# zchuning/repo

Measured on AMD Instinct MI355X. Metric: world-model+imagine updates/sec (B=50,L=50,64x64x3), higher is better.
Workload: dtype f32

## Files before the change

### repo_amd/csrc/dconv.h

```cpp
#pragma once
#include "vgemm.h"

namespace repo {

template <int BM_, int BN_, int CK_, int WM_, int WN_, int LDWPAD_ = 2>
struct DTile {
  static constexpr int BM = BM_, BN = BN_, CK = CK_, WM = WM_, WN = WN_, LDWPAD = LDWPAD_;
  static constexpr int TM = BM / (32 * WM), TN = BN / (32 * WN);
  static constexpr int NT = WM * WN * 64;
  static_assert(TM >= 1 && TN >= 1 && BM % (32 * WM) == 0 && BN % (32 * WN) == 0, "tile / wave grid mismatch");
};

#ifdef REPO_IGEMM_STAMPS
#define REPO_STAMP_FLUSH(nslices)                                              \
  do {                                                                         \
    REPO_STAMP(4);                                                             \
    if ((threadIdx.x & 63) == 0 && blockIdx.x % 16 == 0) {                     \
      for (int i_ = 0; i_ < 6; ++i_) atomicAdd(&g_igemm_stamps[i_], st_[i_]);  \
      atomicAdd(&g_igemm_stamps[6], 1ull);                                     \
      atomicAdd(&g_igemm_stamps[7], (unsigned long long)(nslices));            \
    }                                                                          \
  } while (0)
#else
#define REPO_STAMP_FLUSH(nslices)
#endif

__device__ __forceinline__ int xcd_tile(int b, int n) {
  const int q = n >> 3, r = n & 7, x = b & 7, i = b >> 3;
  return x * q + min(x, r) + i;
}

constexpr int cmin(int a, int b) { return a < b ? a : b; }
constexpr int cmax(int a, int b) { return a > b ? a : b; }

template <class InT>
struct Patch4;
template <>
struct Patch4<float> {
  typedef f32x4 raw_t;
  static constexpr int BYTES = 4;
  static __device__ __forceinline__ raw_t load(__amdgpu_buffer_rsrc_t r, unsigned off) {
    return __builtin_bit_cast(f32x4, __builtin_amdgcn_raw_buffer_load_b128(r, off, 0, 0));
  }
  static __device__ __forceinline__ f32x4 cvt(raw_t v) { return v; }
};
template <>
struct Patch4<uint8_t> {
  typedef unsigned raw_t;
  static constexpr int BYTES = 1;
  static __device__ __forceinline__ raw_t load(__amdgpu_buffer_rsrc_t r, unsigned off) {
    return __builtin_amdgcn_raw_buffer_load_b32(r, off, 0, 0);
  }
  static __device__ __forceinline__ f32x4 cvt(raw_t v) {
    f32x4 o;
    o[0] = pix_norm((uint8_t)(v & 0xff));
    o[1] = pix_norm((uint8_t)((v >> 8) & 0xff));
    o[2] = pix_norm((uint8_t)((v >> 16) & 0xff));
    o[3] = pix_norm((uint8_t)(v >> 24));
    return o;
  }
};

typedef unsigned u32x4s __attribute__((ext_vector_type(4)));

struct DownArgs {
  const void* big;
  const float* w;
  const float* bias;
  const float* aux;
  float* out;
  int nimg, epi;
  unsigned big_bytes, w_bytes;
  float* chan_part;
  unsigned char* cmask;
};

template <class G, class T>
__device__ __forceinline__ void dconv_down_epilogue(const DownArgs& p, float* lds, f32x16 (&acc)[T::TM][T::TN], int n0,
                                                    int m0, int Ntot) {
  constexpr int BM = T::BM, NT = T::NT, TM = T::TM, TN = T::TN;
  constexpr int EP = 36;
  const int tid = threadIdx.x;
  const int lane = tid & 63;
  const int wid = __builtin_amdgcn_readfirstlane(tid >> 6);
  const int wm = wid / T::WN, wn = wid % T::WN;
  const int li = lane & 31, lh = lane >> 5;
  __syncthreads();
  float* strip = lds + wid * 32 * EP;
  const __amdgpu_buffer_rsrc_t rout = make_rsrc(p.out, 4u * (unsigned)Ntot * G::CS);
  float csum[TM][4];
#pragma unroll
  for (int i = 0; i < TM; ++i)
#pragma unroll
    for (int q4 = 0; q4 < 4; ++q4) csum[i][q4] = 0.f;
  const __amdgpu_buffer_rsrc_t raux =
      make_rsrc((p.aux && p.epi != REPO_EPI_FILM_RELU) ? p.aux : p.out, (p.epi == REPO_EPI_MUL_MASK4 ? 1u : 4u) * (unsigned)Ntot * G::CS);
#pragma unroll
  for (int i = 0; i < TM; ++i)
#pragma unroll
    for (int j = 0; j < TN; ++j) {
#pragma unroll
      for (int r = 0; r < 16; ++r) strip[((r & 3) + 8 * (r >> 2) + 4 * lh) * EP + li] = acc[i][j][r];
      __builtin_amdgcn_wave_barrier();
      const int nb = n0 + (wn * TN + j) * 32, mt = m0 + (wm * TM + i) * 32;
#pragma unroll
      for (int pass = 0; pass < 4; ++pass) {
        const int ml = pass * 8 + (lane >> 3), q = lane & 7;
        const int m = mt + ml, n = nb + 4 * q;
        f32x4 v = *reinterpret_cast<const f32x4*>(strip + ml * EP + 4 * q);
        float qs = 0.f;
        if (m < G::CS && n < Ntot) {
          const float bv = p.bias ? p.bias[m] : 0.f;
          const int img = n / G::PS, pix = n % G::PS;
          const unsigned o = (unsigned)((img * G::CS + m) * G::PS + pix);
          if (pix + 3 < G::PS && n + 3 < Ntot) {
            f32x4 a4 = {1.f, 1.f, 1.f, 1.f};
            if (p.epi == REPO_EPI_MUL_DRELU) {
              a4 = __builtin_bit_cast(f32x4, __builtin_amdgcn_raw_buffer_load_b128(raux, 4u * o, 0, 0));
            } else if (p.epi == REPO_EPI_MUL_MASK4) {
              unsigned bits = (unsigned)__builtin_amdgcn_raw_buffer_load_b8(raux, o >> 2, 0, 0) >> (o & 3);
              if (o & 3) bits |= (unsigned)__builtin_amdgcn_raw_buffer_load_b8(raux, (o >> 2) + 1, 0, 0) << (4 - (o & 3));
#pragma unroll
              for (int e = 0; e < 4; ++e) a4[e] = (bits >> e) & 1u ? 1.f : 0.f;
            }
            float fsc = 1.f, fsh = 0.f;
            if (p.epi == REPO_EPI_FILM_RELU) {
              fsc = p.aux[(size_t)(2 * img) * G::CS + m];
              fsh = p.aux[(size_t)(2 * img + 1) * G::CS + m];
            }
#pragma unroll
            for (int e = 0; e < 4; ++e) {
              float x = v[e] + bv;
              if (p.epi == REPO_EPI_RELU) x = fmaxf(x, 0.f);
              else if (p.epi == REPO_EPI_MUL_DRELU || p.epi == REPO_EPI_MUL_MASK4) x = a4[e] > 0.f ? x : 0.f;
              else if (p.epi == REPO_EPI_FILM_RELU) x = fmaxf(fmaf(fsc, x, fsh), 0.f);
              v[e] = x;
            }
            qs = (v[0] + v[1]) + (v[2] + v[3]);
            __builtin_amdgcn_raw_buffer_store_b128(__builtin_bit_cast(u32x4s, v), rout, 4u * o, 0, 0);
          } else {
#pragma unroll
            for (int e = 0; e < 4; ++e) {
              const int ne = n + e;
              if (ne < Ntot) {
                const int oe = ((ne / G::PS) * G::CS + m) * G::PS + ne % G::PS;
                float x = v[e] + bv;
                if (p.epi == REPO_EPI_RELU) x = fmaxf(x, 0.f);
                else if (p.epi == REPO_EPI_FILM_RELU)
                  x = fmaxf(fmaf(p.aux[(size_t)(2 * (ne / G::PS)) * G::CS + m], x, p.aux[(size_t)(2 * (ne / G::PS) + 1) * G::CS + m]), 0.f);
                else if (p.epi == REPO_EPI_MUL_DRELU) x = p.aux[oe] > 0.f ? x : 0.f;
                else if (p.epi == REPO_EPI_MUL_MASK4)
                  x = (reinterpret_cast<const unsigned char*>(p.aux)[oe >> 2] >> (oe & 3)) & 1 ? x : 0.f;
                p.out[oe] = x;
                qs += x;
              }
            }
          }
        }
        if (p.chan_part) {
          qs += __shfl_xor(qs, 1, 64);
          qs += __shfl_xor(qs, 2, 64);
          qs += __shfl_xor(qs, 4, 64);
          csum[i][pass] += qs;
        }
      }
      if (p.cmask) {
        const int cq = lane >> 3, q = lane & 7;
        const int m4 = mt + 4 * cq, n = nb + 4 * q;
        if (m4 < G::CS && n < Ntot) {
          f32x4 rws[4];
          float bq[4];
#pragma unroll
          for (int c = 0; c < 4; ++c) {
            rws[c] = *reinterpret_cast<const f32x4*>(strip + (4 * cq + c) * EP + 4 * q);
            bq[c] = p.bias ? p.bias[m4 + c] : 0.f;
          }
#pragma unroll
          for (int e = 0; e < 4; ++e) {
            const int ne = n + e;
            if (ne < Ntot) {
              unsigned bits = 0;
#pragma unroll
              for (int c = 0; c < 4; ++c) bits |= (rws[c][e] + bq[c] > 0.f ? 1u : 0u) << c;
              p.cmask[((size_t)(ne / G::PS) * (G::CS / 4) + (m4 >> 2)) * G::PS + ne % G::PS] = (unsigned char)bits;
            }
          }
        }
      }
      __builtin_amdgcn_wave_barrier();
    }
  if (p.chan_part) {
    float* red = lds + (NT / 64) * 32 * EP;
    if ((lane & 7) == 0) {
#pragma unroll
      for (int i = 0; i < TM; ++i)
#pragma unroll
        for (int pass = 0; pass < 4; ++pass) red[wid * (TM * 32) + i * 32 + pass * 8 + (lane >> 3)] = csum[i][pass];
    }
    __syncthreads();
    if (tid < BM && m0 + tid < G::CS) {
      const int wmc = tid / (TM * 32), c = tid % (TM * 32);
      float t = 0.f;
#pragma unroll
      for (int x = 0; x < T::WN; ++x) t += red[(wmc * T::WN + x) * (TM * 32) + c];
      p.chan_part[(size_t)blockIdx.x * G::CS + m0 + tid] = t;
    }
  }
}

template <class G, class BigT, class T>
__global__ __launch_bounds__(T::NT) void dconv_down_kernel(DownArgs p) {
  constexpr int BM = T::BM, BN = T::BN, CK = T::CK, NT = T::NT, TM = T::TM, TN = T::TN;
  constexpr int KSL = CK * G::KK;
  constexpr int NSL = G::CB / CK;
  static_assert(G::CB % CK == 0 && KSL % 4 == 0, "channel chunk must divide CB and give k % 4 == 0");
  constexpr int LDW = BM + T::LDWPAD;
  constexpr int ROWS_FULL = 2 * (G::HS - 1) + G::KS;
  constexpr int LENFULL = (ROWS_FULL * G::WB + 3) & ~3;
  constexpr int NIMG_MAX = (BN - 1) / G::PS + 2;
  constexpr int PLMAX = cmin(NIMG_MAX * LENFULL,
                             ((2 * (BN / G::WS + 2) + NIMG_MAX * (G::KS - 2)) * G::WB + 4 * NIMG_MAX + 3) & ~3);
  constexpr int PLV = PLMAX / 4;
  constexpr int W_NV = BM * KSL / 4, W_KV = KSL / 4;
  constexpr int W_PER = (W_NV + NT - 1) / NT, P_PER = (CK * PLV + NT - 1) / NT;
  constexpr int NBUF = NSL > 1 ? 2 : 1;
  constexpr int EP = 36;
  __shared__ __attribute__((aligned(16))) float lds[cmax(NBUF * KSL * LDW + NBUF * CK * PLMAX, (NT / 64) * 32 * EP + (NT / 64) * TM * 32)];
  float* Wl = lds;
  float* Pl = lds + NBUF * KSL * LDW;

  const int tid = threadIdx.x;
  const int lane = tid & 63;
  const int wid = __builtin_amdgcn_readfirstlane(tid >> 6);
  const int wm = wid / T::WN, wn = wid % T::WN;
  const int li = lane & 31, lh = lane >> 5;

  const int Ntot = p.nimg * G::PS;
  const int n0 = xcd_tile(blockIdx.x, gridDim.x) * BN, m0 = blockIdx.y * BM;
  const int nlast = min(n0 + BN, Ntot) - 1;
  const int ia = n0 / G::PS, ib = nlast / G::PS;
  const int fa = (n0 % G::PS) / G::WS, lb = (nlast % G::PS) / G::WS;
  const int la_ = (ia == ib) ? lb : G::HS - 1;
  const int lenA = ((2 * (la_ - fa) + G::KS) * G::WB + 3) & ~3;
  auto span_start = [&](int i) __attribute__((always_inline)) { return i == ia ? 0 : lenA + (i - ia - 1) * LENFULL; };
  const int PL = span_start(ib) + (ib == ia ? lenA : ((2 * lb + G::KS) * G::WB + 3) & ~3);

  const __amdgpu_buffer_rsrc_t rbig = make_rsrc(p.big, p.big_bytes), rw = make_rsrc(p.w, p.w_bytes);

  unsigned woff[W_PER];
  int wlds[W_PER];
#pragma unroll
  for (int j = 0; j < W_PER; ++j) {
    const int v = tid + j * NT, kv = v % W_KV, m = v / W_KV;
    const bool act = (W_NV % NT == 0) || v < W_NV;
    woff[j] = act ? 4u * (unsigned)(min(m0 + m, G::CS - 1) * (G::CB * G::KK) + kv * 4) : kOobOffset;
    wlds[j] = act ? (kv * 4) * LDW + m : -1;
  }
  unsigned poff[P_PER];
  int plds[P_PER];
#pragma unroll
  for (int j = 0; j < P_PER; ++j) {
    const int v = tid + j * NT, c = v / PLV, q = (v % PLV) * 4;
    const bool act = c < CK && q < PL;
    int i, rel;
    if (q < lenA) {
      i = ia;
      rel = q;
    } else {
      i = ia + 1 + (q - lenA) / LENFULL;
      rel = (q - lenA) % LENFULL;
    }
    const int f = (i == ia) ? fa : 0;
    poff[j] = act ? (unsigned)Patch4<BigT>::BYTES * (unsigned)((i * G::CB + c) * G::PB + 2 * f * G::WB + rel)
                  : kOobOffset;
    plds[j] = act ? c * PLMAX + q : -1;
  }
  constexpr unsigned W_STEP = 4u * KSL, P_STEP = (unsigned)Patch4<BigT>::BYTES * CK * G::PB;

  int bbase[TN];
#pragma unroll
  for (int j = 0; j < TN; ++j) {
    const int n = min(n0 + (wn * TN + j) * 32 + li, Ntot - 1);
    const int i = n / G::PS, pix = n % G::PS;
    const int f = (i == ia) ? fa : 0;
    bbase[j] = span_start(i) + 2 * (pix / G::WS - f) * G::WB + 2 * (pix % G::WS);
  }
  int bbase1[TN];
#pragma unroll
  for (int j = 0; j < TN; ++j) bbase1[j] = bbase[j] + lh;
  const int abase = lh * LDW + wm * (TM * 32) + li;

  f32x16 acc[TM][TN];
#pragma unroll
  for (int i = 0; i < TM; ++i)
#pragma unroll
    for (int j = 0; j < TN; ++j)
#pragma unroll
      for (int r = 0; r < 16; ++r) acc[i][j][r] = 0.f;

  f32x4 rwv[W_PER];
  typename Patch4<BigT>::raw_t rpv[P_PER];
  auto gload = [&](int t) __attribute__((always_inline)) {
#pragma unroll
    for (int j = 0; j < W_PER; ++j)
      rwv[j] = VecLoad<4>::load(rw, woff[j] == kOobOffset ? kOobOffset : woff[j] + (unsigned)t * W_STEP);
#pragma unroll
    for (int j = 0; j < P_PER; ++j)
      rpv[j] = Patch4<BigT>::load(rbig, poff[j] == kOobOffset ? kOobOffset : poff[j] + (unsigned)t * P_STEP);
  };
  auto lstore = [&](int buf) __attribute__((always_inline)) {
    float* wl = Wl + buf * KSL * LDW;
    float* pl = Pl + buf * CK * PLMAX;
#pragma unroll
    for (int j = 0; j < W_PER; ++j)
      if ((W_NV % NT == 0) || wlds[j] >= 0) {
#pragma unroll
        for (int e = 0; e < 4; ++e) wl[wlds[j] + e * LDW] = rwv[j][e];
      }
#pragma unroll
    for (int j = 0; j < P_PER; ++j)
      if (plds[j] >= 0) *reinterpret_cast<f32x4*>(pl + plds[j]) = Patch4<BigT>::cvt(rpv[j]);
  };
  auto koff = [](int k) constexpr { return (k / G::KK) * PLMAX + ((k % G::KK) / G::KS) * G::WB + (k % G::KK) % G::KS; };
  auto compute = [&](int buf) __attribute__((always_inline)) {
    const float* wl = Wl + buf * KSL * LDW + abase;
    const float* pl = Pl + buf * CK * PLMAX;
#pragma unroll
    for (int ks = 0; ks < KSL / 2; ++ks) {
      const int o0 = koff(2 * ks), o1 = koff(2 * ks + 1);
      float av[TM], bv[TN];
#pragma unroll
      for (int i = 0; i < TM; ++i) av[i] = wl[2 * ks * LDW + i * 32];
#pragma unroll
      for (int j = 0; j < TN; ++j) bv[j] = (o1 == o0 + 1) ? pl[bbase1[j] + o0] : pl[bbase[j] + (lh ? o1 : o0)];
#pragma unroll
      for (int i = 0; i < TM; ++i)
#pragma unroll
        for (int j = 0; j < TN; ++j)
          acc[i][j] = __builtin_amdgcn_mfma_f32_32x32x2f32(av[i], bv[j], acc[i][j], 0, 0, 0);
    }
  };

  REPO_STAMP_DECL
  gload(0);
  lstore(0);
  __syncthreads();
  REPO_STAMP(5);
  if (NSL == 1) {
    compute(0);
  } else {
    int buf = 0;
    for (int t = 0; t < NSL; ++t) {
      gload(min(t + 1, NSL - 1));
      __builtin_amdgcn_sched_barrier(0);
      REPO_STAMP(0);
      compute(buf);
      __builtin_amdgcn_sched_barrier(0);
      REPO_STAMP(1);
      lstore(buf ^ 1);
      REPO_STAMP(2);
      __syncthreads();
      REPO_STAMP(3);
      buf ^= 1;
    }
  }

  dconv_down_epilogue<G, T>(p, lds, acc, n0, m0, Ntot);
  REPO_STAMP_FLUSH(NSL);
}

template <class G, class BigT, class T>
inline int launch_dconv_down(const DownArgs& a, hipStream_t s) {
  const long gx = ((long)a.nimg * G::PS + T::BN - 1) / T::BN, gy = (G::CS + T::BM - 1) / T::BM;
  hipLaunchKernelGGL((dconv_down_kernel<G, BigT, T>), dim3((unsigned)gx, (unsigned)gy), dim3(T::NT), 0, s, a);
  hipError_t e = hipGetLastError();
  return e == hipSuccess ? REPO_OK : (int)e;
}

struct WgradArgs {
  const float* small;
  const void* big;
  float* slab;
  int nimg, imgs_per_split, want_db;
  unsigned small_bytes, big_bytes;
  int nsplits_tw = 0;
  int want_dbig = 0;
};

template <int BM_, int BN_, int WM_, int WN_, int GI_, int RB_, int SPREAD_ = 0>
struct WTile {
  static constexpr int BM = BM_, BN = BN_, WM = WM_, WN = WN_, GI = GI_, RB = RB_, SPREAD = SPREAD_;
  static constexpr int TM = BM / (32 * WM), TN = BN / (32 * WN), NT = WM * WN * 64;
  static_assert(TM >= 1 && TN >= 1 && BM % (32 * WM) == 0 && BN % (32 * WN) == 0, "tile / wave grid mismatch");
};

constexpr int pitch4(int len) {
  int p = (len + 3) & ~3;
  return (p / 4) % 2 ? p : p + 4;
}

template <class G, class BigT, class T>
__global__ __launch_bounds__(T::NT) void dconv_wgrad_kernel(WgradArgs p) {
  constexpr int BM = T::BM, BN = T::BN, TM = T::TM, TN = T::TN, NT = T::NT, GI = T::GI, RB = T::RB;
  constexpr int NW = G::CB * G::KK;
  constexpr int NB = (G::HS + RB - 1) / RB;
  constexpr int BR = 2 * RB + G::KS - 2;
  constexpr int BRP = (G::WB % 64 == 0) ? G::WB + 4 : G::WB;
  constexpr int ALEN = RB * G::WS, BLEN = BR * BRP;
  constexpr int AP = pitch4(ALEN), BP = pitch4(BLEN);
  constexpr int CBT = cmin(G::CB, (BN + G::KK - 2) / G::KK + 1);
  constexpr int A_VPC = (ALEN + 3) / 4, B_VPC = (BR * G::WB + 3) / 4;
  constexpr int A_NV = GI * BM * A_VPC, B_NV = GI * CBT * B_VPC;
  constexpr int A_PER = (A_NV + NT - 1) / NT, B_PER = (B_NV + NT - 1) / NT;
  constexpr int SXP = (G::WS + 1) / 2;
  __shared__ __attribute__((aligned(16))) float lds[GI * BM * AP + GI * CBT * BP + 64];
  float* Al = lds;
  float* Bl = lds + GI * BM * AP;

  const int tid = threadIdx.x;
  const int lane = tid & 63;
  const int wid = __builtin_amdgcn_readfirstlane(tid >> 6);
  const int wm = wid / T::WN, wn = wid % T::WN;
  const int li = lane & 31, lh = lane >> 5;

  int bx = blockIdx.x, by = blockIdx.y, z = blockIdx.z;
  {
    const int tpz = gridDim.x * gridDim.y, gz = gridDim.z;
    const int L = bx + gridDim.x * (by + gridDim.y * z);
    const int full = (gz / 8) * 8 * tpz;
    if (L < full) {
      const int grp = L / (8 * tpz), r = L % (8 * tpz);
      const int t = r / 8;
      z = grp * 8 + r % 8;
      bx = t % (int)gridDim.x;
      by = t / (int)gridDim.x;
    }
  }
  const int n0 = bx * BN, m0 = by * BM;
  const int img_beg = z * p.imgs_per_split, img_end = min(p.nimg, img_beg + p.imgs_per_split);
  const int cbf = n0 / G::KK;
  const int ngrp = (img_end - img_beg + GI - 1) / GI;
  const int nch = ngrp * NB;

  const __amdgpu_buffer_rsrc_t rsm = make_rsrc(p.small, p.small_bytes), rbg = make_rsrc(p.big, p.big_bytes);

  int aoff[A_PER], boff[B_PER], ag[A_PER], bg[B_PER];
  int alds[A_PER], blds[B_PER];
#pragma unroll
  for (int j = 0; j < A_PER; ++j) {
    const int v = tid + j * NT, e4 = v % A_VPC, rm = v / A_VPC;
    const int m = rm % BM, g = rm / BM;
    const bool act = g < GI && m0 + m < G::CS;
    ag[j] = act ? g : 1 << 20;
    aoff[j] = (g * G::CS + m0 + m) * G::PS + e4 * 4;
    alds[j] = (g * BM + m) * AP + e4 * 4;
  }
#pragma unroll
  for (int j = 0; j < B_PER; ++j) {
    const int v = tid + j * NT, e4 = v % B_VPC, rc = v / B_VPC;
    const int c = rc % CBT, g = rc / CBT;
    const bool act = g < GI && cbf + c < G::CB;
    bg[j] = act ? g : 1 << 20;
    boff[j] = (g * G::CB + cbf + c) * G::PB + e4 * 4;
    blds[j] = (g * CBT + c) * BP + (BRP == G::WB ? e4 * 4 : (e4 * 4 / G::WB) * BRP + e4 * 4 % G::WB);
  }

  int abase[TM], bbase[TN];
#pragma unroll
  for (int i = 0; i < TM; ++i) abase[i] = ((wm * TM + i) * 32 + li) * AP + lh;
#pragma unroll
  for (int j = 0; j < TN; ++j) {
    const int n = min(n0 + (wn * TN + j) * 32 + li, NW - 1);
    const int cb = n / G::KK, r = n % G::KK;
    bbase[j] = (cb - cbf) * BP + (r / G::KS) * BRP + r % G::KS + 2 * lh;
  }

  f32x16 acc[TM][TN];
#pragma unroll
  for (int i = 0; i < TM; ++i)
#pragma unroll
    for (int j = 0; j < TN; ++j)
#pragma unroll
      for (int r = 0; r < 16; ++r) acc[i][j][r] = 0.f;
  float dbsum = 0.f;

  f32x4 rav[A_PER];
  typename Patch4<BigT>::raw_t rbv[B_PER];
  constexpr int NLD = A_PER + B_PER;
  int ld_img0 = 0, ld_abias = 0, ld_bbias = 0;
  auto gload_begin = [&](int c) __attribute__((always_inline)) {
    const int grp = c / NB, band = c % NB;
    const int r0 = band * RB;
    ld_img0 = img_beg + grp * GI;
    ld_abias = ld_img0 * G::CS * G::PS + r0 * G::WS;
    ld_bbias = ld_img0 * G::CB * G::PB + 2 * r0 * G::WB;
  };
  auto gload_piece = [&](int q) __attribute__((always_inline)) {
#pragma unroll
    for (int j = 0; j < A_PER; ++j)
      if (j == q)
        rav[j] = VecLoad<4>::load(rsm, ld_img0 + ag[j] < img_end ? 4u * (unsigned)(aoff[j] + ld_abias) : kOobOffset);
#pragma unroll
    for (int j = 0; j < B_PER; ++j)
      if (j + A_PER == q)
        rbv[j] = Patch4<BigT>::load(
            rbg, ld_img0 + bg[j] < img_end ? (unsigned)Patch4<BigT>::BYTES * (unsigned)(boff[j] + ld_bbias) : kOobOffset);
  };
  auto gload = [&](int c) __attribute__((always_inline)) {
    gload_begin(c);
#pragma unroll
    for (int q = 0; q < NLD; ++q) gload_piece(q);
  };
  auto lstore = [&]() __attribute__((always_inline)) {
#pragma unroll
    for (int j = 0; j < A_PER; ++j)
      if ((A_NV % NT == 0) || tid + j * NT < A_NV) *reinterpret_cast<f32x4*>(Al + alds[j]) = rav[j];
#pragma unroll
    for (int j = 0; j < B_PER; ++j)
      if ((B_NV % NT == 0) || tid + j * NT < B_NV) *reinterpret_cast<f32x4*>(Bl + blds[j]) = Patch4<BigT>::cvt(rbv[j]);
  };
  int bbase_w[TN];
#pragma unroll
  for (int j = 0; j < TN; ++j) bbase_w[j] = bbase[j] - 2 * lh + lh * (2 * BRP - 2 * G::WS + 2);
  constexpr int RL = G::HS - (NB - 1) * RB;
  auto compute = [&](auto rows_tag, int c) __attribute__((always_inline)) {
    constexpr int ROWS = decltype(rows_tag)::value;
    constexpr int NK = ROWS * G::WS, NP = (NK + 1) / 2;
    const int band = c % NB;
    const int R = min(RB, G::HS - band * RB);
#pragma unroll
    for (int g = 0; g < GI; ++g) {
      const float* ar = Al + g * BM * AP;
      const float* br = Bl + g * CBT * BP;
#pragma unroll
      for (int pp = 0; pp < NP; ++pp) {
        const int k0 = 2 * pp;
        const int off0 = 2 * (k0 / G::WS) * BRP + 2 * (k0 % G::WS);
        const bool straddle = (k0 % G::WS) == G::WS - 1;
        const bool half = k0 + 1 >= NK;
        float av[TM], bv[TN];
#pragma unroll
        for (int i = 0; i < TM; ++i) {
          av[i] = ar[abase[i] + k0];
          if (half) av[i] = lh ? 0.f : av[i];
        }
#pragma unroll
        for (int j = 0; j < TN; ++j) {
          bv[j] = (straddle && !half) ? br[bbase_w[j] + off0] : br[bbase[j] + off0];
          if (half) bv[j] = lh ? 0.f : bv[j];
        }
#pragma unroll
        for (int i = 0; i < TM; ++i)
#pragma unroll
          for (int j = 0; j < TN; ++j)
            acc[i][j] = __builtin_amdgcn_mfma_f32_32x32x2f32(av[i], bv[j], acc[i][j], 0, 0, 0);
        constexpr int NSLOT = GI * NP;
        constexpr int SSLOT = (NSLOT + cmax(T::SPREAD, 1) - 1) / cmax(T::SPREAD, 1);
        const int slot = g * NP + pp;
        if (T::SPREAD && slot < SSLOT && slot * NLD / SSLOT < (slot + 1) * NLD / SSLOT) {
          __builtin_amdgcn_sched_barrier(0);
#pragma unroll
          for (int q = slot * NLD / SSLOT; q < (slot + 1) * NLD / SSLOT; ++q) gload_piece(q);
          __builtin_amdgcn_sched_barrier(0);
        }
      }
    }
    if (p.want_db && bx == 0) {
      constexpr int PARTS = NT / BM;
      const int m = tid % BM, part = tid / BM;
      if (part < PARTS) {
        for (int g = 0; g < GI; ++g)
          for (int e = part; e < R * G::WS; e += PARTS) dbsum += Al[(g * BM + m) * AP + e];
      }
    }
  };

  REPO_STAMP_DECL
  if (nch > 0) {
    gload(0);
    REPO_STAMP(5);
    for (int c = 0; c < nch; ++c) {
      lstore();
      REPO_STAMP(2);
      __syncthreads();
      REPO_STAMP(3);
      gload_begin(min(c + 1, nch - 1));
      if (!T::SPREAD) {
#pragma unroll
        for (int q = 0; q < NLD; ++q) gload_piece(q);
        __builtin_amdgcn_sched_barrier(0);
      }
      REPO_STAMP(0);
      if (RL == RB || c % NB != NB - 1) compute(std::integral_constant<int, RB>{}, c);
      else compute(std::integral_constant<int, RL>{}, c);
      REPO_STAMP(1);
      __syncthreads();
      REPO_STAMP(3);
    }
  }

  constexpr int LDS_ = NW + 1;
#pragma unroll
  for (int i = 0; i < TM; ++i)
#pragma unroll
    for (int j = 0; j < TN; ++j) {
      const int n = n0 + (wn * TN + j) * 32 + li;
      const int mb = m0 + (wm * TM + i) * 32 + 4 * lh;
      if (n < NW && mb < G::CS) {
        float* cdst = p.slab + ((size_t)z * G::CS + mb) * LDS_ + n;
#pragma unroll
        for (int r = 0; r < 16; ++r) {
          const int dm = (r & 3) + 8 * (r >> 2);
          if (mb + dm < G::CS) cdst[dm * LDS_] = acc[i][j][r];
        }
      }
    }
  if (p.want_db && bx == 0) {
    constexpr int PARTS = NT / BM;
    float* red = lds;
    red[tid] = dbsum;
    __syncthreads();
    if (tid < BM && m0 + tid < G::CS) {
      float s = 0.f;
      for (int q = 0; q < PARTS; ++q) s += red[q * BM + tid];
      p.slab[((size_t)z * G::CS + m0 + tid) * LDS_ + NW] = s;
    }
  }
  REPO_STAMP_FLUSH(nch);
}

template <class G, class BigT, class T>
inline int launch_dconv_wgrad(const WgradArgs& a, int splits, hipStream_t s) {
  constexpr int NW = G::CB * G::KK;
  dim3 grid((NW + T::BN - 1) / T::BN, (G::CS + T::BM - 1) / T::BM, (unsigned)splits);
  hipLaunchKernelGGL((dconv_wgrad_kernel<G, BigT, T>), grid, dim3(T::NT), 0, s, a);
  hipError_t e = hipGetLastError();
  return e == hipSuccess ? REPO_OK : (int)e;
}

struct NllArgs {
  const float* h3;
  const float* w;
  const float* bias;
  const void* target;
  float* recon;
  float* dpre;
  unsigned char* mask4;
  float* partials;
  float grad_scale;
  int nimg;
  unsigned h3_bytes;
  float* chan_partials = nullptr;
};

typedef float f32x4acc __attribute__((ext_vector_type(4)));

template <class TgtT>
__global__ __launch_bounds__(256) __attribute__((amdgpu_waves_per_eu(2))) void dconv_dec4_nll_kernel(NllArgs p) {
  constexpr int CS = 32, HS = 30, PS = 900, HB = 64, PP = 34, PLANE = 400, ROWS = 10;
  constexpr int NVEC = CS * 75, P_PER = (NVEC + 255) / 256;
  __shared__ __attribute__((aligned(16))) float lds[9 * 8 * 64 + CS * PLANE];
  __shared__ float red[16];
  float* Wf = lds;
  float* Pl = lds + 9 * 8 * 64;

  const int tid = threadIdx.x;
  const int lane = tid & 63;
  const int wv = __builtin_amdgcn_readfirstlane(tid >> 6);
  const int lj = lane & 15, lg = lane >> 4;
  const int ntiles = p.nimg * 4;

  for (int i = tid; i < 9 * 8 * 64; i += 256) {
    const int l = i & 63, cq = (i >> 6) & 7, tap = i >> 9;
    const int m = l & 15, c = 4 * cq + (l >> 4);
    float v = 0.f;
    if (m < 12) {
      const int py = m / 6, cb = (m % 6) >> 1, px = m & 1;
      const int ky = py + 2 * (2 - tap / 3), kx = px + 2 * (2 - tap % 3);
      v = p.w[((c * 3 + cb) * 6 + ky) * 6 + kx];
    }
    Wf[i] = v;
  }
  for (int i = tid; i < CS * PLANE / 4; i += 256) reinterpret_cast<f32x4*>(Pl)[i] = f32x4{0.f, 0.f, 0.f, 0.f};

  const __amdgpu_buffer_rsrc_t rh = make_rsrc(p.h3, p.h3_bytes);
  int pgo[P_PER];
  int ppk[P_PER];
  unsigned long long mtop = 0ull, mbot = 0ull;
#pragma unroll
  for (int j = 0; j < P_PER; ++j) {
    const int v = tid + j * 256, c = v / 75, e4 = v % 75;
    const bool act = v < NVEC;
    pgo[j] = act ? c * PS + e4 * 4 : -1;
    const int q0 = e4 * 4;
    ppk[j] = (c * PLANE + (q0 / 30) * PP + q0 % 30 + 2) | ((q0 % 30) << 16);
#pragma unroll
    for (int e = 0; e < 4; ++e) {
      const int r = (q0 + e) / 30;
      if (r < 2) mtop |= 1ull << (j * 4 + e);
      if (r >= 8) mbot |= 1ull << (j * 4 + e);
    }
  }
  int bbase[4];
#pragma unroll
  for (int t = 0; t < 4; ++t) bbase[t] = lg * PLANE + (2 * wv + (t >> 1)) * PP + 16 * (t & 1) + lj;

  f32x4 rpv[P_PER];
  auto gload = [&](int tile) __attribute__((always_inline)) {
    const int img = tile >> 2, cy0 = (tile & 3) * 8;
    const int bias_ = img * CS * PS + (cy0 - 2) * HS;
#pragma unroll
    for (int j = 0; j < P_PER; ++j)
      rpv[j] = VecLoad<4>::load(rh, pgo[j] >= 0 ? 4u * (unsigned)(pgo[j] + bias_) : kOobOffset);
  };
  auto lstore = [&](int tile) __attribute__((always_inline)) {
    const int rg = tile & 3;
    const unsigned long long bad = (rg == 0 ? mtop : 0ull) | (rg == 3 ? mbot : 0ull);
    const int e4_end = rg == 3 ? 60 : 75;
    const long mbase = (long)(tile >> 2) * CS * PS + ((tile & 3) * 8 - 2) * HS;
#pragma unroll
    for (int j = 0; j < P_PER; ++j)
      if (pgo[j] >= 0) {
        if (p.mask4) {
          const int v = tid + j * 256, e4 = v % 75;
          if (e4 >= 15 && e4 < e4_end) {
            const unsigned nib = (rpv[j][0] > 0.f ? 1u : 0u) | (rpv[j][1] > 0.f ? 2u : 0u) | (rpv[j][2] > 0.f ? 4u : 0u) |
                                 (rpv[j][3] > 0.f ? 8u : 0u);
            p.mask4[(mbase + pgo[j]) >> 2] = (unsigned char)nib;
          }
        }
        const int base = ppk[j] & 0xffff, col0 = ppk[j] >> 16;
#pragma unroll
        for (int e = 0; e < 4; ++e)
          Pl[base + e + (col0 + e >= 30 ? PP - 30 : 0)] = ((bad >> (j * 4 + e)) & 1ull) ? 0.f : rpv[j][e];
      }
  };

  float lsum = 0.f;
  const int G = gridDim.x;
  int tile = blockIdx.x;
  if (tile < ntiles) gload(tile);
  __syncthreads();
  for (; tile < ntiles; tile += G) {
    lstore(tile);
    __syncthreads();
    if (tile + G < ntiles) gload(tile + G);
    __builtin_amdgcn_sched_barrier(0);

    f32x4acc acc[4];
#pragma unroll
    for (int t = 0; t < 4; ++t) acc[t] = f32x4acc{0.f, 0.f, 0.f, 0.f};
#pragma unroll
    for (int tap = 0; tap < 9; ++tap)
#pragma unroll
      for (int cq = 0; cq < 8; ++cq) {
        const float a = Wf[(tap * 8 + cq) * 64 + lane];
#pragma unroll
        for (int t = 0; t < 4; ++t) {
          const float b = Pl[bbase[t] + 4 * cq * PLANE + (tap / 3) * PP + tap % 3];
          acc[t] = __builtin_amdgcn_mfma_f32_16x16x4f32(a, b, acc[t], 0, 0, 0);
        }
      }

    const int img = tile >> 2, cy0 = (tile & 3) * 8;
    if (lg < 3) {
      const int odd = lj & 1;
      const int q = 2 * lg + odd, py = q / 3, cb = q % 3;
      const float bv = p.bias ? p.bias[cb] : 0.f;
#pragma unroll
      for (int t = 0; t < 4; ++t) {
        const float k0 = odd ? acc[t][2] : acc[t][0], k1 = odd ? acc[t][3] : acc[t][1];
        const float s0 = odd ? acc[t][0] : acc[t][2], s1 = odd ? acc[t][1] : acc[t][3];
        const float r0 = __shfl_xor(s0, 1, 64), r1 = __shfl_xor(s1, 1, 64);
        const float v0 = (odd ? r0 : k0) + bv, v1 = (odd ? r1 : k1) + bv, v2 = (odd ? k0 : r0) + bv, v3 = (odd ? k1 : r1) + bv;
        const int cy = cy0 + 2 * wv + (t >> 1), cx = 16 * (t & 1) + lj;
        const int o = ((img * 3 + cb) * HB + 2 * cy + py) * HB + 4 * (cx >> 1);
        float t0, t1, t2, t3;
        if (sizeof(TgtT) == 1) {
          const unsigned tw = *reinterpret_cast<const unsigned*>((const uint8_t*)p.target + o);
          t0 = pix_norm((uint8_t)(tw & 0xff));
          t1 = pix_norm((uint8_t)((tw >> 8) & 0xff));
          t2 = pix_norm((uint8_t)((tw >> 16) & 0xff));
          t3 = pix_norm((uint8_t)(tw >> 24));
        } else {
          const float4 tw = *reinterpret_cast<const float4*>((const float*)p.target + o);
          t0 = tw.x, t1 = tw.y, t2 = tw.z, t3 = tw.w;
        }
        const float d0 = v0 - t0, d1 = v1 - t1, d2 = v2 - t2, d3 = v3 - t3;
        lsum += 0.5f * ((d0 * d0 + d1 * d1) + (d2 * d2 + d3 * d3));
        if (p.dpre)
          *reinterpret_cast<float4*>(p.dpre + o) = make_float4(d0 * p.grad_scale, d1 * p.grad_scale, d2 * p.grad_scale, d3 * p.grad_scale);
        if (p.recon) *reinterpret_cast<float4*>(p.recon + o) = make_float4(v0, v1, v2, v3);
      }
    }
    __syncthreads();
  }
  const float s = block_sum(lsum, red);
  if (tid == 0) p.partials[blockIdx.x] = s;
}

inline int dec4_nll_grid(long nimg) {
  const long ntiles = nimg * 4;
  return (int)(ntiles < 1024 ? ntiles : 1024);
}

}
```

Measured before the change: 172.9.

## Software-pipeline LDS fragment fetches and fold bias-grad sum into MFMA loop

Restructures the wgrad compute loop so each step's LDS operand loads are issued one step ahead into a double buffer, with scheduling barriers separating fetch from MFMA issue. The bias-gradient row sum is interleaved into the MFMA slots with a small lookahead, instead of running as a separate serial loop afterwards. The A tile pitch becomes odd, so A stores are done as scalar writes rather than 16-byte vector writes, aiming to cut LDS bank conflicts on reads. In exchange, register pressure rises, and the bias sum now reads LDS in every block, not only when it is needed.

```diff
diff --git a/repo_amd/csrc/dconv.h b/repo_amd/csrc/dconv.h
--- a/repo_amd/csrc/dconv.h
+++ b/repo_amd/csrc/dconv.h
@@ -407,9 +407,9 @@
   constexpr int BR = 2 * RB + G::KS - 2;
   constexpr int BRP = (G::WB % 64 == 0) ? G::WB + 4 : G::WB;
   constexpr int ALEN = RB * G::WS, BLEN = BR * BRP;
-  constexpr int AP = pitch4(ALEN), BP = pitch4(BLEN);
   constexpr int CBT = cmin(G::CB, (BN + G::KK - 2) / G::KK + 1);
   constexpr int A_VPC = (ALEN + 3) / 4, B_VPC = (BR * G::WB + 3) / 4;
+  constexpr int AP = 4 * A_VPC + 1, BP = pitch4(BLEN);
   constexpr int A_NV = GI * BM * A_VPC, B_NV = GI * CBT * B_VPC;
   constexpr int A_PER = (A_NV + NT - 1) / NT, B_PER = (B_NV + NT - 1) / NT;
   constexpr int SXP = (G::WS + 1) / 2;
@@ -514,7 +514,13 @@
   auto lstore = [&]() __attribute__((always_inline)) {
 #pragma unroll
     for (int j = 0; j < A_PER; ++j)
-      if ((A_NV % NT == 0) || tid + j * NT < A_NV) *reinterpret_cast<f32x4*>(Al + alds[j]) = rav[j];
+      if ((A_NV % NT == 0) || tid + j * NT < A_NV) {
+        if (AP % 4 == 0) *reinterpret_cast<f32x4*>(Al + alds[j]) = rav[j];
+        else {
+#pragma unroll
+          for (int e = 0; e < 4; ++e) Al[alds[j] + e] = rav[j][e];
+        }
+      }
 #pragma unroll
     for (int j = 0; j < B_PER; ++j)
       if ((B_NV % NT == 0) || tid + j * NT < B_NV) *reinterpret_cast<f32x4*>(Bl + blds[j]) = Patch4<BigT>::cvt(rbv[j]);
@@ -523,56 +529,87 @@
 #pragma unroll
   for (int j = 0; j < TN; ++j) bbase_w[j] = bbase[j] - 2 * lh + lh * (2 * BRP - 2 * G::WS + 2);
   constexpr int RL = G::HS - (NB - 1) * RB;
-  auto compute = [&](auto rows_tag, int c) __attribute__((always_inline)) {
+  constexpr int PARTS = NT / BM;
+  const int dm = tid % BM, dpart = tid / BM;
+  const float* dbrow = Al + dm * AP + dpart;
+  auto compute = [&](auto rows_tag) __attribute__((always_inline)) {
     constexpr int ROWS = decltype(rows_tag)::value;
     constexpr int NK = ROWS * G::WS, NP = (NK + 1) / 2;
-    const int band = c % NB;
-    const int R = min(RB, G::HS - band * RB);
-#pragma unroll
-    for (int g = 0; g < GI; ++g) {
-      const float* ar = Al + g * BM * AP;
-      const float* br = Bl + g * CBT * BP;
-#pragma unroll
-      for (int pp = 0; pp < NP; ++pp) {
-        const int k0 = 2 * pp;
-        const int off0 = 2 * (k0 / G::WS) * BRP + 2 * (k0 % G::WS);
-        const bool straddle = (k0 % G::WS) == G::WS - 1;
-        const bool half = k0 + 1 >= NK;
-        float av[TM], bv[TN];
-#pragma unroll
-        for (int i = 0; i < TM; ++i) {
-          av[i] = ar[abase[i] + k0];
-          if (half) av[i] = lh ? 0.f : av[i];
-        }
-#pragma unroll
-        for (int j = 0; j < TN; ++j) {
-          bv[j] = (straddle && !half) ? br[bbase_w[j] + off0] : br[bbase[j] + off0];
-          if (half) bv[j] = lh ? 0.f : bv[j];
-        }
-#pragma unroll
-        for (int i = 0; i < TM; ++i)
+    constexpr int D = TM * TN >= 2 ? 1 : 0, NFB = D + 1;
+    constexpr int NSLOT = GI * NP, U = D ? 2 : 1, NST = (NSLOT + U - 1) / U;
+    float fa[NFB][U][TM], fb[NFB][U][TN];
+    auto fetch = [&](int t) __attribute__((always_inline)) {
+#pragma unroll
+      for (int u = 0; u < U; ++u) {
+        const int s = t * U + u;
+        if (s < NSLOT) {
+          const int g = s / NP, k0 = 2 * (s % NP);
+          const float* ar = Al + g * BM * AP;
+          const float* br = Bl + g * CBT * BP;
+          const int off0 = 2 * (k0 / G::WS) * BRP + 2 * (k0 % G::WS);
+          const bool straddle = (k0 % G::WS) == G::WS - 1;
+          const bool half = k0 + 1 >= NK;
+#pragma unroll
+          for (int i = 0; i < TM; ++i) fa[t % NFB][u][i] = ar[abase[i] + k0];
 #pragma unroll
           for (int j = 0; j < TN; ++j)
-            acc[i][j] = __builtin_amdgcn_mfma_f32_32x32x2f32(av[i], bv[j], acc[i][j], 0, 0, 0);
-        constexpr int NSLOT = GI * NP;
-        constexpr int SSLOT = (NSLOT + cmax(T::SPREAD, 1) - 1) / cmax(T::SPREAD, 1);
-        const int slot = g * NP + pp;
-        if (T::SPREAD && slot < SSLOT && slot * NLD / SSLOT < (slot + 1) * NLD / SSLOT) {
-          __builtin_amdgcn_sched_barrier(0);
-#pragma unroll
-          for (int q = slot * NLD / SSLOT; q < (slot + 1) * NLD / SSLOT; ++q) gload_piece(q);
-          __builtin_amdgcn_sched_barrier(0);
-        }
-      }
-    }
-    if (p.want_db && bx == 0) {
-      constexpr int PARTS = NT / BM;
-      const int m = tid % BM, part = tid / BM;
-      if (part < PARTS) {
-        for (int g = 0; g < GI; ++g)
-          for (int e = part; e < R * G::WS; e += PARTS) dbsum += Al[(g * BM + m) * AP + e];
-      }
-    }
+            fb[t % NFB][u][j] = (straddle && !half) ? br[bbase_w[j] + off0] : br[bbase[j] + off0];
+        }
+      }
+    };
+    constexpr int NE = (NK + PARTS - 1) / PARTS, NDB = GI * NE, DLA = 4;
+    float dbv[DLA];
+    auto dbread = [&](int q) __attribute__((always_inline)) {
+      const int g = q / NE, i = q % NE;
+      const bool all = (i + 1) * PARTS <= NK;
+      return dbrow[g * BM * AP + (all ? i * PARTS : min(i * PARTS, NK - 1 - dpart))];
+    };
+    auto dbadd = [&](int q) __attribute__((always_inline)) {
+      const int i = q % NE;
+      if ((i + 1) * PARTS <= NK || dpart + i * PARTS < NK) dbsum += dbv[q % DLA];
+      if (q + DLA < NDB) dbv[q % DLA] = dbread(q + DLA);
+    };
+    {
+#pragma unroll
+      for (int q = 0; q < DLA; ++q)
+        if (q < NDB) dbv[q] = dbread(q);
+    }
+#pragma unroll
+    for (int t = 0; t < D; ++t)
+      if (t < NST) fetch(t);
+#pragma unroll
+    for (int t = 0; t < NST; ++t) {
+      if (t + D < NST) fetch(t + D);
+      if (D) __builtin_amdgcn_sched_barrier(0);
+#pragma unroll
+      for (int u = 0; u < U; ++u) {
+        const int slot = t * U + u;
+        if (slot < NSLOT) {
+          const bool half = 2 * (slot % NP) + 1 >= NK;
+          float av[TM], bv[TN];
+#pragma unroll
+          for (int i = 0; i < TM; ++i) av[i] = half && lh ? 0.f : fa[t % NFB][u][i];
+#pragma unroll
+          for (int j = 0; j < TN; ++j) bv[j] = half && lh ? 0.f : fb[t % NFB][u][j];
+#pragma unroll
+          for (int i = 0; i < TM; ++i)
+#pragma unroll
+            for (int j = 0; j < TN; ++j)
+              acc[i][j] = __builtin_amdgcn_mfma_f32_32x32x2f32(av[i], bv[j], acc[i][j], 0, 0, 0);
+          if (slot < NDB) dbadd(slot);
+          constexpr int SSLOT = (NSLOT + cmax(T::SPREAD, 1) - 1) / cmax(T::SPREAD, 1);
+          if (T::SPREAD && slot < SSLOT && slot * NLD / SSLOT < (slot + 1) * NLD / SSLOT) {
+            __builtin_amdgcn_sched_barrier(0);
+#pragma unroll
+            for (int q = slot * NLD / SSLOT; q < (slot + 1) * NLD / SSLOT; ++q) gload_piece(q);
+            __builtin_amdgcn_sched_barrier(0);
+          }
+        }
+      }
+      if (D) __builtin_amdgcn_sched_barrier(0);
+    }
+#pragma unroll
+    for (int q = NSLOT; q < NDB; ++q) dbadd(q);
   };
 
   REPO_STAMP_DECL
@@ -591,8 +628,8 @@
         __builtin_amdgcn_sched_barrier(0);
       }
       REPO_STAMP(0);
-      if (RL == RB || c % NB != NB - 1) compute(std::integral_constant<int, RB>{}, c);
-      else compute(std::integral_constant<int, RL>{}, c);
+      if (RL == RB || c % NB != NB - 1) compute(std::integral_constant<int, RB>{});
+      else compute(std::integral_constant<int, RL>{});
       REPO_STAMP(1);
       __syncthreads();
       REPO_STAMP(3);
@@ -616,7 +653,6 @@
       }
     }
   if (p.want_db && bx == 0) {
-    constexpr int PARTS = NT / BM;
     float* red = lds;
     red[tid] = dbsum;
     __syncthreads();
```

Result: no change. 172.8 (-0.0%).
